# sm-edwards/CrossScale-ECG-A-Modular-HPC-Pipeline-from-Locality-Optimization-to-MPI-GPU-Overlap

Measured on AMD Instinct MI355X. Metric: ECG samples/sec (node) + conv1d speedup vs torch.Conv1d, tiny 1D-CNN at 1/2/4/8 GPU, higher is better.
Workload: dtype bf16; 1 GPU; model=TinyECG (1458 params), global_batch=256, seq_len=500, parallelism=dp1, sync=fedavg every 50 local steps (none all_reduce AVG, overlap=none), per_client_batch=256, max_windows_per_client=20000, backend=fused

## Files before the change

### crossscale-ecg-a-modular-hpc-pipeline-from-locality-optimization-to-mpi-gpu-overlap_amd/ops/_lib.py

```python
from __future__ import annotations

import ctypes as C
import os
import threading
from typing import Optional

import torch

LIB_DIR = os.environ.get("ECG_LIB_DIR") or os.path.join(os.path.dirname(os.path.dirname(os.path.abspath(__file__))), "_lib")

_lock = threading.Lock()
_libs = {}

vp, i32, i64, f32 = C.c_void_p, C.c_int, C.c_long, C.c_float
u64 = C.c_uint64
f64p = C.POINTER(C.c_double)
i32p = C.POINTER(C.c_int)
i64p = C.POINTER(C.c_int64)

STATUS = {0: "ok", 1: "bad argument", 2: "problem too large for the fused kernel", 3: "HIP runtime error",
          4: "I/O error", 5: "timeout", 6: "end of data"}


class NativeError(RuntimeError):
# ... 10 lines not shown
        if name in _libs:
            return _libs[name]
        path = os.path.join(LIB_DIR, name)
        lib = None
        if os.path.exists(path):
            lib = C.CDLL(path, mode=C.RTLD_GLOBAL)
        _libs[name] = lib
        return lib


def _sig(lib, name, argtypes, restype=i32):
    fn = getattr(lib, name)
    fn.argtypes = argtypes
    fn.restype = restype
    return fn


class TinyRound(C.Structure):
    _fields_ = [("X", vp), ("ldx", i64), ("idx", vp), ("Y", vp), ("params", vp), ("mom", vp), ("slab", vp),
                ("loss_acc", vp), ("wprep", vp), ("xg", vp), ("yg", vp),
                ("L", i32), ("nc", i32), ("slab_stride", i32), ("B", i32), ("steps", i32),
                ("lr", f32), ("momentum", f32), ("wd", f32), ("nesterov", i32), ("prec", i32),
                ("dp_clip", f32), ("dp_sigma", f32), ("dp_seed", u64), ("dp_scale", vp), ("dp_step", vp),
                ("xbg", vp)]


class TinyCohortRound(C.Structure):
    _fields_ = [("X", vp), ("ldx", i64), ("idx", vp), ("Y", vp), ("params", vp), ("mom", vp), ("slab", vp),
                ("loss_acc", vp), ("wprep", vp), ("xg", vp), ("yg", vp), ("xbg", vp), ("global_params", vp),
                ("L", i32), ("nc", i32), ("slab_stride", i32), ("B", i32), ("steps", i32), ("M", i32),
                ("fanout", i32), ("lr", f32), ("momentum", f32), ("wd", f32), ("nesterov", i32), ("prec", i32),
                ("cdp_clip", f32), ("cdp_sigma", f32), ("server_lr", f32), ("cdp_seed", u64), ("cdp_scale", vp),
                ("cdp_norm", vp), ("cdp_round", vp), ("server_opt", i32), ("server_beta1", f32), ("server_beta2", f32),
                ("server_tau", f32), ("server_m", vp), ("server_v", vp)]


def _bind_kernels(lib: C.CDLL) -> None:
    _sig(lib, "ecg_tiny_param_count", [i32])
    _sig(lib, "ecg_tiny_smem_bytes", [i32, i32])
    _sig(lib, "ecg_tiny_step_grads", [vp, i32, i64, vp, vp, vp, i32, vp, i32, i32, f32, i32, vp, vp])
    _sig(lib, "ecg_tiny_forward", [vp, i32, i64, vp, vp, i32, vp, i32, i32, vp, vp])
    _sig(lib, "ecg_tiny_wprep_bytes", [])
    _sig(lib, "ecg_tiny_prep", [vp, vp, vp])
    _sig(lib, "ecg_tiny_eval", [vp, i32, i64, vp, vp, i32, vp, i32, vp, vp, vp, vp, vp, i32, vp])
    _sig(lib, "ecg_tiny_eval_scratch_bytes", [i32])
    _sig(lib, "ecg_tiny_eval_out_bytes", [i32])
    _sig(lib, "ecg_slab_reduce_sgd", [vp, i32, i32, i32, vp, vp, vp, vp, f32, f32, f32, i32, i32, vp, vp])
    _sig(lib, "ecg_slab_reduce_dp_sgd", [vp, i32, i32, i32, vp, vp, vp, vp, f32, f32, f32, i32, i32, vp,
                                         f32, f32, u64, vp, vp, vp])
    _sig(lib, "ecg_dp_noise", [vp, i32, u64, u64, vp])
    native = _sig(lib, "ecg_tiny_round_sizeof", [])()
    if native != C.sizeof(TinyRound):
        raise NativeError(f"EcgTinyRound is {native} bytes in libecg_kernels.so but {C.sizeof(TinyRound)} in "
                          "ops/_lib.py: rebuild the library (python csrc/build.py) or update TinyRound")
    _sig(lib, "ecg_tiny_round_enqueue", [C.POINTER(TinyRound), vp])
    _sig(lib, "ecg_tiny_round_capture", [C.POINTER(vp), C.POINTER(TinyRound)])
    native = _sig(lib, "ecg_tiny_cohort_round_sizeof", [])()
    if native != C.sizeof(TinyCohortRound):
        raise NativeError(f"EcgTinyCohortRound is {native} bytes in libecg_kernels.so but {C.sizeof(TinyCohortRound)} "
                          "in ops/_lib.py: rebuild the library (python csrc/build.py) or update TinyCohortRound")
    _sig(lib, "ecg_tiny_cohort_round_enqueue", [C.POINTER(TinyCohortRound), vp])
    _sig(lib, "ecg_tiny_cohort_round_capture", [C.POINTER(vp), C.POINTER(TinyCohortRound)])
    _sig(lib, "ecg_cohort_dp_close", [vp, vp, i32, i32, f32, f32, f32, u64, vp, vp, vp, vp])
    _sig(lib, "ecg_cohort_dp_noise", [vp, i32, u64, u64, vp])
    _sig(lib, "ecg_cohort_server_close", [vp, vp, i32, i32, f32, f32, f32, u64, vp, vp, vp, i32, f32, f32, f32, vp, vp,
                                          vp])
    _sig(lib, "ecg_tiny_cohort_param_stride", [i32])
    _sig(lib, "ecg_tiny_cohort_wprep_stride", [])
    _sig(lib, "ecg_tiny_gather_floats", [i32, i32], i64)
    _sig(lib, "ecg_tiny_gather_halfs", [i32, i32], i64)
    _sig(lib, "ecg_tiny_step_grads_twice", [vp, i32, i64, vp, vp, vp, i32, vp, i32, i32, f32, i32, vp, vp])
    _sig(lib, "ecg_tiny_force_waves", [i32])
    _sig(lib, "ecg_tiny_set_stamps", [vp])
    _sig(lib, "ecg_round_graph_launch", [vp, vp])
    _sig(lib, "ecg_round_graph_destroy", [vp])
    _sig(lib, "ecg_round_graph_upload", [vp, vp])
    _sig(lib, "conv1d_batch_hip", [vp, vp, vp, i32, i32, i32, vp])
    _sig(lib, "conv1d_batch_hip_sync", [vp, vp, vp, i32, i32, i32, vp])
    _sig(lib, "conv1d_batch_hip_spin", [vp, vp, vp, i32, i32, i32, vp])
    _sig(lib, "conv1d_batch_hip_flag", [vp, vp, vp, i32, i32, i32, vp])
    _sig(lib, "conv1d_valid_dgrad_hip", [vp, vp, vp, i32, i32, i32, vp])
    _sig(lib, "conv1d_valid_dgrad_hip_bf16", [vp, vp, vp, i32, i32, i32, vp])
    _sig(lib, "conv1d_valid_wgrad_ws_floats", [i32, i32, i32], i64)
    _sig(lib, "conv1d_valid_wgrad_hip", [vp, vp, vp, vp, i64, i32, i32, i32, vp])
    _sig(lib, "conv1d_valid_wgrad_hip_bf16", [vp, vp, vp, vp, i64, i32, i32, i32, vp])
    _sig(lib, "conv1d_batch_hip_bf16", [vp, vp, vp, i32, i32, i32, vp])
    _sig(lib, "ecg_sgd_flat", [vp, vp, vp, i64, f32, f32, f32, f32, i32, i32, f32, vp, vp])
    _sig(lib, "ecg_gather_rows_f32", [vp, i64, i32, vp, i32, vp, i64, i32, f32, vp])
    _sig(lib, "ecg_gather_rows_bf16", [vp, i64, i32, vp, i32, vp, i64, i32, f32, vp])
    for extra in ("_bind_conv_mc",):
        fn = globals().get(extra)
        if fn:
            fn(lib)
# ... 91 lines not shown
```

### crossscale-ecg-a-modular-hpc-pipeline-from-locality-optimization-to-mpi-gpu-overlap_amd/ops/fused_tiny.py

```python
from __future__ import annotations

import ctypes as C
import os
from typing import Optional

import torch

from . import _lib
from ..models.tiny_ecg import TinyECG, num_params
from ..data.dataset import DeviceIndexSampler
from ..utils.philox import mix64
from .tiny_eval import EvalResult, TinyEvaluator, evaluate_torch, tiny_evaluate


PRECISION = {"bf16": 0, "fp32": 1}


def prec_id(precision: str) -> int:
    if precision not in PRECISION:
        raise ValueError(f"precision must be one of {list(PRECISION)}, got {precision!r}")
    return PRECISION[precision]


def new_wprep(device) -> torch.Tensor:
# ... 49 lines not shown
    _lib.check(st, "ecg_tiny_forward")
    return out


def tiny_step_grads(flat_params: torch.Tensor, x: torch.Tensor, y32: torch.Tensor, idx: Optional[torch.Tensor],
                    batch: int, num_classes: int = 2, slab: Optional[torch.Tensor] = None,
                    precision: str = "bf16", prefrag: bool = True,
                    wprep: Optional[torch.Tensor] = None) -> torch.Tensor:
    _check_dataset(x, y32, num_classes)
    if idx is not None:
        _check_idx(idx, batch, x.shape[0], x.device)
    stride = slab_stride(num_classes)
    if slab is None:
        slab = torch.empty((batch, stride), dtype=torch.float32, device=x.device)
    lib = _lib.kernels()
    wp, _keep = _wprep_ptr(precision, prefrag, x.device, wprep)
    st = lib.ecg_tiny_step_grads(x.data_ptr(), x.shape[1], x.stride(0), _lib.ptr(idx), y32.data_ptr(),
                                 flat_params.data_ptr(), num_classes, slab.data_ptr(), stride, batch,
                                 1.0 / batch, prec_id(precision), wp, _lib.stream_ptr(x.device))
    _lib.check(st, "ecg_tiny_step_grads")
    return slab


def check_dp_args(dp_clip: float, dp_noise: float) -> None:
    if not dp_clip >= 0.0 or not dp_noise >= 0.0:
        raise ValueError(f"dp_clip and dp_noise must be >= 0, got {dp_clip} and {dp_noise}")
    if dp_noise > 0.0 and dp_clip == 0.0:
        raise ValueError("dp_noise > 0 needs a clip norm (dp_clip > 0): the noise is scaled by it")


def dp_reduce_slab(slab: torch.Tensor, dp_clip: float, dp_noise: float, dp_seed: int, dp_step: torch.Tensor,
                   num_classes: int = 2):
    P = num_params(num_classes)
    grad = torch.empty(P, dtype=torch.float32, device=slab.device)
    loss = torch.zeros(1, dtype=torch.float32, device=slab.device)
    scale = torch.empty(slab.shape[0], dtype=torch.float32, device=slab.device)
    st = _lib.kernels().ecg_slab_reduce_dp_sgd(
        slab.data_ptr(), slab.shape[0], slab.stride(0), P, None, None, grad.data_ptr(), loss.data_ptr(), 0.0, 0.0, 0.0,
        0, 0, None, dp_clip, dp_noise, int(dp_seed) & (2 ** 64 - 1), scale.data_ptr(), dp_step.data_ptr(),
        _lib.stream_ptr(slab.device))
    _lib.check(st, "ecg_slab_reduce_dp_sgd")
    return grad, loss, scale


def dp_noise(P: int, seed: int, t: int, device) -> torch.Tensor:
    z = torch.empty(P, dtype=torch.float32, device=device)
    st = _lib.kernels().ecg_dp_noise(z.data_ptr(), P, int(seed) & (2 ** 64 - 1), int(t) & (2 ** 64 - 1),
                                     _lib.stream_ptr(z.device))
    _lib.check(st, "ecg_dp_noise")
    return z


def reduce_slab(slab: torch.Tensor, num_classes: int = 2):
    P = num_params(num_classes)
    grad = torch.empty(P, dtype=torch.float32, device=slab.device)
    loss = torch.zeros(1, dtype=torch.float32, device=slab.device)
    lib = _lib.kernels()
    st = lib.ecg_slab_reduce_sgd(slab.data_ptr(), slab.shape[0], slab.shape[1], P, None, None, grad.data_ptr(),
                                 loss.data_ptr(), 0.0, 0.0, 0.0, 0, 0, None, _lib.stream_ptr(slab.device))
    _lib.check(st, "ecg_slab_reduce_sgd")
    return grad, loss


class FusedTinyTrainer:

    def __init__(self, model: TinyECG, x_gpu: torch.Tensor, y_gpu: torch.Tensor, batch_size: int,
                 steps_per_round: int, lr: float = 1e-2, momentum: float = 0.9, weight_decay: float = 0.0,
                 nesterov: bool = False, seed: Optional[int] = None, use_graph: Optional[bool] = None,
                 precision: str = "bf16", prefrag: bool = True, gather: bool = True, pack: bool = True,
                 dp_clip: float = 0.0, dp_noise: float = 0.0, dp_seed: Optional[int] = None):
        self.device = x_gpu.device
        self.precision = precision
        self.prec = prec_id(precision)
        self.model = model
        self.nc = model.num_classes
        self.params = model.flat if model.flat is not None else model.flatten_parameters()
        if self.params.device != self.device:
            raise ValueError("model and dataset must be on the same device")
        self.P = num_params(self.nc)
        self.x = x_gpu.contiguous()
        self.y32 = labels_int32(y_gpu, self.nc)
        _check_dataset(self.x, self.y32, self.nc)
        self.B = int(batch_size)
        self.S = int(steps_per_round)
        self.lr, self.momentum, self.wd, self.nesterov = float(lr), float(momentum), float(weight_decay), bool(nesterov)
        self.stride = slab_stride(self.nc)
        self.mom = torch.zeros_like(self.params)
        self.slab = torch.empty((self.B, self.stride), dtype=torch.float32, device=self.device)
        self.loss_acc = torch.zeros(1, dtype=torch.float32, device=self.device)
        self.idx_table = torch.zeros((self.S, self.B), dtype=torch.int32, device=self.device)
        self.idx_stage = torch.zeros((self.S, self.B), dtype=torch.int32, device=self.device)
        self._staged: Optional[int] = None
        self._loss_steps = 0
        self.sampler = DeviceIndexSampler(self.x.shape[0], self.B, self.device, seed=seed)
        self.use_graph = (os.environ.get("ECG_TINY_GRAPH", "1") != "0") if use_graph is None else bool(use_graph)
        self._graphs = {}
        self.steps_done = 0
        self._evaluator: Optional[TinyEvaluator] = None
        lib = _lib.kernels()
        L = self.x.shape[1]
        smem = lib.ecg_tiny_smem_bytes(L, self.prec)
        if smem > 160 * 1024:
            raise ValueError(f"window length {L} too long for the fused kernel ({smem} B LDS)")
        self.prefrag = bool(prefrag) and precision == "bf16"
        self.wprep = new_wprep(self.device) if self.prefrag else None
        self.gather = bool(gather) and self.prefrag
        self.xg = self.yg = None
        if self.gather:
            self.xg = torch.zeros(lib.ecg_tiny_gather_floats(L, self.B), dtype=torch.float32, device=self.device)
            self.yg = torch.zeros(2 * self.B, dtype=torch.int32, device=self.device)
        self.pack = bool(pack) and self.gather
        self.xbg = None
        if self.pack:
            self.xbg = torch.zeros(lib.ecg_tiny_gather_halfs(L, self.B), dtype=torch.bfloat16, device=self.device)
        check_dp_args(dp_clip, dp_noise)
        self.dp_clip, self.dp_noise = float(dp_clip), float(dp_noise)
        self.dp = self.dp_clip > 0.0
        self.dp_seed = (mix64(0 if seed is None else seed) if dp_seed is None else int(dp_seed)) & (2 ** 64 - 1)
        self.dp_steps = 0
        self.dp_scale = self.dp_step = None
        if self.dp:
            self.dp_scale = torch.zeros(self.B, dtype=torch.float32, device=self.device)
            self.dp_step = torch.zeros(1, dtype=torch.int64, device=self.device)
        self._round = _lib.TinyRound(
            X=self.x.data_ptr(), ldx=self.x.stride(0), Y=self.y32.data_ptr(), params=self.params.data_ptr(),
            mom=self.mom.data_ptr(), slab=self.slab.data_ptr(), loss_acc=self.loss_acc.data_ptr(),
            wprep=_lib.ptr(self.wprep), xg=_lib.ptr(self.xg), yg=_lib.ptr(self.yg), L=L, nc=self.nc,
            slab_stride=self.stride, B=self.B, lr=self.lr, momentum=self.momentum, wd=self.wd,
            nesterov=int(self.nesterov), prec=self.prec, dp_clip=self.dp_clip, dp_sigma=self.dp_noise,
            dp_seed=self.dp_seed, dp_scale=_lib.ptr(self.dp_scale), dp_step=_lib.ptr(self.dp_step),
            xbg=_lib.ptr(self.xbg))

    def _round_of(self, n: int, table: torch.Tensor):
        r = self._round
        r.idx, r.steps = table.data_ptr(), n
        return C.byref(r)

    def _graph_for(self, n: int, table: torch.Tensor) -> C.c_void_p:
        key = (n, table.data_ptr())
        g = self._graphs.get(key)
        if g is None:
            g = C.c_void_p()
            torch.cuda.synchronize(self.device)
            _lib.check(_lib.kernels().ecg_tiny_round_capture(C.byref(g), self._round_of(n, table)),
                       "ecg_tiny_round_capture")
            self._graphs[key] = g
        return g

    def close(self):
        graphs, self._graphs = getattr(self, "_graphs", {}), {}
        for g in graphs.values():
            if g.value:
                _lib.kernels().ecg_round_graph_destroy(g)

# ... 100 lines not shown
```

### csrc/kernels/tiny_ecg_step.hip

```cpp
#include "../include/ecg_common.h"
#include "../include/tiny_ecg.h"

#include <cfloat>
#include <climits>
#include <cstdint>
#include <cstdlib>
#include <cstring>
#include <type_traits>

namespace {

using namespace ecg::tiny;

constexpr int MAX_PAIRS_PER_WAVE = 4;

struct Smem {
  int Lp;
  int xs_off, xcol_off, h1_off, dh2_off, ps_off, frag_off, red_off, bytes;
};

constexpr int RED_G = 0;
constexpr int RED_POOLED = 16;
constexpr int RED_POOL = 48;

struct FusedOpt {
  int slab_wt;
};
__host__ __device__ constexpr int msplit(int waves) { return (waves - 1) / 5 < 1 ? 1 : (waves - 1) / 5; }
__host__ __device__ constexpr int red_cnt(int waves) { return RED_POOL + waves * 16; }
__host__ __device__ constexpr int red_m(int waves) { return red_cnt(waves) + waves * 16; }
__host__ __device__ constexpr int red_dw1(int waves) { return red_m(waves) + msplit(waves) * 1280; }
__host__ __device__ constexpr int red_head(int waves) { return red_dw1(waves) + waves * 128; }
__host__ __device__ constexpr int red_floats(int waves) { return red_head(waves) + 288; }

typedef unsigned u32x4 __attribute__((ext_vector_type(4)));
typedef unsigned u32x2 __attribute__((ext_vector_type(2)));

__device__ __forceinline__ void st_wt(__amdgpu_buffer_rsrc_t r, int idx, float v) {
  __builtin_amdgcn_raw_buffer_store_b32(__builtin_bit_cast(unsigned, v), r, idx * 4, 0, 16);
}
__device__ __forceinline__ void st_wt4(__amdgpu_buffer_rsrc_t r, int idx, f32x4 v) {
  typedef int i32x4 __attribute__((ext_vector_type(4)));
  __builtin_amdgcn_raw_buffer_store_b128(__builtin_bit_cast(i32x4, v), r, idx * 4, 0, 16);
}
__device__ __forceinline__ void st_wt_b64(__amdgpu_buffer_rsrc_t r, int byte_off, u32x2 v) {
  __builtin_amdgcn_raw_buffer_store_b64(v, r, byte_off, 0, 16);
}
__device__ __forceinline__ void st_wt_b16(__amdgpu_buffer_rsrc_t r, int byte_off, unsigned short v) {
  __builtin_amdgcn_raw_buffer_store_b16(v, r, byte_off, 0, 16);
}
__device__ __forceinline__ float ld_wt(__amdgpu_buffer_rsrc_t r, int idx) {
  return __builtin_bit_cast(float, __builtin_amdgcn_raw_buffer_load_b32(r, idx * 4, 0, 16));
}
constexpr int kOobByte = 0x40000000;

constexpr int kPackLead = 4;
__host__ __device__ constexpr int pack_ldb(int L) { return (L + 31) / 32 * 32 + 8; }

constexpr int F32_KSTEPS = C * K2 / 4;

__host__ __device__ constexpr bool frag_pad_is_bias(int which, int l, int j) { return which == 0 && j == 0 && l < 48; }

__device__ __forceinline__ void wprep_put(unsigned char* wp, int i, float v) {
  __bf16* wb = reinterpret_cast<__bf16*>(wp);
  if (i < C * K1) {
    wb[WP_AW1 + (i / K1) * 8 + i % K1] = ecg::to_bf16(v);
// ... 714 lines not shown
    }
  }
};

__host__ __device__ constexpr int cohort_pstride(int P) { return (P + 63) / 64 * 64; }
constexpr int kCohortWprepStride = (WP_BYTES + 127) / 128 * 128;

template <int WAVES, int MODE, bool F32, bool PF, bool PK = false>
__global__ __launch_bounds__(WAVES * 64) void tiny_ecg_step_kernel(
    const float* __restrict__ X, long ldx,
    const unsigned char* __restrict__ wprep,
    const int* __restrict__ Y,
    unsigned long long* __restrict__ stamps,
    int L, int nc,
    const float* __restrict__ params,
    float* __restrict__ out, int out_stride,
    float inv_B,
    const int* __restrict__ idx,
    int slab_wt) {
  extern __shared__ __attribute__((aligned(16))) unsigned char smem[];
  TinySample<WAVES, F32, PF, PK> S(smem, L, nc);
  constexpr bool TRAIN = MODE != 1;
  constexpr bool COHORT = MODE == 3;
  const int tid = threadIdx.x;
  const int b = COHORT ? blockIdx.y * gridDim.x + blockIdx.x : blockIdx.x;
  const long rows = COHORT ? (long)gridDim.x * gridDim.y : (long)gridDim.x;
  if constexpr (COHORT) {
    params += (long)blockIdx.y * cohort_pstride(S.lay.P);
    if constexpr (PF) wprep += (long)blockIdx.y * kCohortWprepStride;
  }
  const __amdgpu_buffer_rsrc_t slab_r = make_rsrc(out, rows * out_stride * 4);
  const int rowbase = b * out_stride;
  if (stamps && tid == 0) stamps[(long)b * 16 + 15] = __builtin_amdgcn_s_memrealtime();
#pragma unroll 1
  for (int rep = 0; rep < (MODE == 2 ? 2 : 1); ++rep) {
#define ECG_STAMP(k) \
  if (stamps && tid == 0) stamps[(long)b * 16 + 7 * rep + (k)] = __builtin_amdgcn_s_memtime();
    ECG_STAMP(0)
    int ylab = 0;
    long row = b;
    if constexpr (!PK) row = idx ? (long)idx[b] : (long)b;
    const float* xrow = X + row * ldx;
    [[maybe_unused]] const __amdgpu_buffer_rsrc_t xr = make_rsrc(xrow, PK ? ldx * 4 : (long)L * 4);
    [[maybe_unused]] typename TinySample<WAVES, F32, PF, PK>::X1 x0;
    [[maybe_unused]] float hv_pk = 0.f;
    if constexpr (PK) {
      S.conv1_load(xr, 0, x0);
      ylab = Y[row];
      S.pf_load_fwd(wprep);
      const int i = S.lay.wh + tid;
      hv_pk = i < S.lay.P ? params[i] : 0.f;
    } else if constexpr (PF) {
      S.pf_load_fwd(wprep);
      const int i = S.lay.wh + tid;
      const float hv = i < S.lay.P ? params[i] : 0.f;
      if (TRAIN) ylab = Y[row];
      S.conv1_load(xr, 0, x0);
      if (i < S.lay.P) S.ps[i] = hv;
      static_assert(MAX_CLASSES * C + MAX_CLASSES <= 8 * 64, "head parameters: one per thread");
    } else {
      constexpr int PR = 4;
      float pv[PR];
#pragma unroll
      for (int j = 0; j < PR; ++j) {
        const int i = tid + j * S.NT;
        pv[j] = i < S.lay.P ? params[i] : 0.f;
// ... 13 lines not shown
      for (int i = tid + PR * S.NT; i < S.lay.P; i += S.NT) S.put_param(i, params[i]);
    }
    S.zero_pads();
    if constexpr (F32) {
      __syncthreads();
      ECG_STAMP(1)
      S.conv1();
    } else {
      ECG_STAMP(1)
      S.conv1_mfma(xr, x0);
      if constexpr (PK) {
        const int i = S.lay.wh + tid;
        if (i < S.lay.P) S.ps[i] = hv_pk;
      }
    }
    __syncthreads();
    ECG_STAMP(2)
    S.conv2();
    if constexpr (PF && TRAIN) S.pf_load_dgrad(wprep);
    __syncthreads();
    ECG_STAMP(3)
    S.template head_and_M<TRAIN>(ylab, inv_B, out, out_stride, b);
    if (!TRAIN) return;
    if (MODE == 0 && stamps && (tid & 63) == 0 && (S.w <= 1 || S.w == WAVES - 1))
      stamps[(long)b * 16 + 8 + (S.w == 0 ? 0 : S.w == 1 ? 1 : 2)] = __builtin_amdgcn_s_memtime();
    __syncthreads();
    ECG_STAMP(4)
    S.dgrad();
    __syncthreads();
    ECG_STAMP(5)
    if (WAVES == 16 && slab_wt && S.lay.P - S.lay.b2 + 1 <= S.NT - 448) {
      S.row_store(slab_r, rowbase);
    } else if (slab_wt) {
      for (int i = tid; i <= S.lay.P; i += S.NT) st_wt(slab_r, rowbase + i, S.row_value(i));
    } else {
      for (int i = tid; i <= S.lay.P; i += S.NT) out[rowbase + i] = S.row_value(i);
    }
    ECG_STAMP(6)
#undef ECG_STAMP
    if (MODE == 2) __syncthreads();
  }
  if (stamps && tid == 0) stamps[(long)b * 16 + 14] = __builtin_amdgcn_s_memrealtime();
}

constexpr int kRedColsDefault = 32;
constexpr int kRedApply = 1, kRedNesterov = 2;
inline int red_flags(int apply, int nesterov) { return (apply ? kRedApply : 0) | (nesterov ? kRedNesterov : 0); }
constexpr int RED_ROWG = 16;

struct GatherArgs {
  const float* X;
  long ldx;
  const int* idx;
  const int* Y;
  float* xg;
  int* yg;
  int L, ldg, B, vec;
  __bf16* xbg;
  int ldb;
};
__host__ __device__ inline int gather_rows_per_block(int L, int vec, int nt) {
  const int per_row = vec ? L / 4 : L;
  return per_row >= nt ? 1 : nt / per_row;
}

template <int NT>
__device__ __forceinline__ void gather_block(const GatherArgs& ga, int nred) {
  const int per_row = ga.vec ? ga.L / 4 : ga.L;
  const int rpb = gather_rows_per_block(ga.L, ga.vec, NT);
  const int r0 = ((int)blockIdx.x - nred) * rpb;
  const __amdgpu_buffer_rsrc_t xr = make_rsrc(ga.xg, (long)ga.B * ga.ldg * 4);
  const __amdgpu_buffer_rsrc_t br = make_rsrc(ga.xbg, ga.xbg ? (long)ga.B * ga.ldb * 2 : 0);
  const int npad = ga.ldb - ga.L;
  for (int e = threadIdx.x; e < rpb * per_row; e += NT) {
    const int lr_ = e / per_row, j = e - lr_ * per_row, b = r0 + lr_;
    if (b >= ga.B) break;
    const long row = ga.idx[b];
    if (ga.vec) {
      const f32x4 v = *reinterpret_cast<const f32x4*>(ga.X + row * ga.ldx + 4 * j);
      st_wt4(xr, b * ga.ldg + 4 * j, v);
      if (ga.xbg) {
        bf16x4 p;
#pragma unroll
        for (int q = 0; q < 4; ++q) p[q] = ecg::to_bf16(v[q]);
        st_wt_b64(br, (b * ga.ldb + kPackLead + 4 * j) * 2, __builtin_bit_cast(u32x2, p));
        for (int u = j; u < npad / 4; u += per_row)
          st_wt_b64(br, (b * ga.ldb + (u == 0 ? 0 : ga.L + 4 * u)) * 2, u32x2{0u, 0u});
      }
    } else {
      const float v = ga.X[row * ga.ldx + j];
      st_wt(xr, b * ga.ldg + j, v);
      if (ga.xbg) {
        st_wt_b16(br, (b * ga.ldb + kPackLead + j) * 2, __builtin_bit_cast(unsigned short, ecg::to_bf16(v)));
        for (int u = j; u < npad; u += per_row)
          st_wt_b16(br, (b * ga.ldb + (u < kPackLead ? u : ga.L + u)) * 2, (unsigned short)0);
// ... 231 lines not shown
  if (lane == 0) {
    const float n = sqrtf(ss);
    norm[c] = n;
    scale[c] = n > 0.f ? fminf(1.f, clip / n) : 1.f;
  }
}

template <int NT>
__global__ __launch_bounds__(NT) void cohort_dp_mean_kernel(
    const float* __restrict__ params, float* __restrict__ global_params, int P, int M, float inv_M,
    const float* __restrict__ scale, float server_lr, float noise_scale, unsigned long long seed,
    const unsigned long long* __restrict__ round_word) {
  const int i = blockIdx.x * NT + threadIdx.x;
  if (i >= P) return;
  const int pstride = cohort_pstride(P);
  float noise = 0.f;
  if (noise_scale != 0.f) noise = noise_scale * cohort_dp_normal(i, seed, round_word[0] - 1ull);
  const float g = global_params[i];
  float s = scale[0] * (params[i] - g);
  for (int c = 1; c < M; ++c) s += scale[c] * (params[(long)c * pstride + i] - g);
  global_params[i] = g + server_lr * (s * inv_M + noise);
}

unsigned long long* g_stamps = nullptr;

FusedOpt no_fuse() {
  FusedOpt o{};
  o.slab_wt = 1;
  return o;
}

struct StepArgs {
  const float* X;
  int L;
  long ldx;
  const int* idx;
  const int* Y;
  const float* params;
  int nc;
  float* out;
  int out_stride, B;
  float inv_B;
  const unsigned char* wprep;
  bool packed = false;
};

template <int WAVES, int MODE, bool F32, bool PF, bool PK = false>
int launch_step(const StepArgs& a, hipStream_t stream, int M = 1) {
  const Smem sm = make_smem(a.L, WAVES, a.nc, F32);
  auto kern = tiny_ecg_step_kernel<WAVES, MODE, F32, PF, PK>;
  if (sm.bytes > 64 * 1024)
    ECG_HIP_CHECK(hipFuncSetAttribute((const void*)kern, hipFuncAttributeMaxDynamicSharedMemorySize, sm.bytes));
  if (PK && a.idx) return ecg::kBadArg;
  hipLaunchKernelGGL(kern, dim3(a.B, M), dim3(WAVES * 64), sm.bytes, stream, a.X, a.ldx, PF ? a.wprep : nullptr, a.Y,
                     g_stamps, a.L, a.nc, a.params, a.out, a.out_stride, a.inv_B, a.idx, no_fuse().slab_wt);
  ECG_HIP_CHECK(hipGetLastError());
  return ecg::kOk;
}

int launch_prep(const float* params, unsigned char* wprep, hipStream_t stream) {
  if (!params || !wprep) return ecg::kBadArg;
  hipLaunchKernelGGL(tiny_prep_kernel, dim3(1), dim3(256), 0, stream, params, wprep);
  ECG_HIP_CHECK(hipGetLastError());
  return ecg::kOk;
}

constexpr int kMaxLds = 160 * 1024;

int g_forced_waves = 0;
int pick_waves(int L, bool f32) {
  const int Lp = (L + 31) / 32 * 32;
  const int forced = g_forced_waves;
  const bool fit16 = Lp <= 32 * 4 * 16 && make_smem(L, 16, MAX_CLASSES, f32).bytes <= kMaxLds;
  if (forced == 16 && fit16) return 16;
  if (forced == 8) return 8;
  return (fit16 && Lp / 32 >= 16) ? 16 : 8;
}
// ... 3 lines not shown
  const int Lp = (L + 31) / 32 * 32;
  if (Lp > 32 * 4 * 8 || make_smem(L, 8, MAX_CLASSES, f32).bytes > kMaxLds) return ecg::kTooLarge;
  const Layout lay = make_layout(nc);
  if (mode != 1 && out_stride < lay.P + 1) return ecg::kBadArg;
  if (mode == 1 && out_stride < nc) return ecg::kBadArg;
  return ecg::kOk;
}

template <bool F32, bool PF>
int dispatch_cfg(int mode, int waves, const StepArgs& a, hipStream_t stream) {
  if (mode == 2)
    return launch_step<8, 2, F32, PF>(a, stream);
  if (mode == 0) return waves == 8 ? launch_step<8, 0, F32, PF>(a, stream) : launch_step<16, 0, F32, PF>(a, stream);
  return waves == 8 ? launch_step<8, 1, F32, PF>(a, stream) : launch_step<16, 1, F32, PF>(a, stream);
}

int step_dispatch(int mode, int prec, const StepArgs& a, hipStream_t stream) {
  if (prec != 0 && prec != 1) return ecg::kBadArg;
  int st = check_step_args(a.L, a.nc, a.B, a.out_stride, mode, prec == 1);
  if (st) return st;
  if (a.wprep && prec == 1) return ecg::kBadArg;
  const int waves = pick_waves(a.L, prec == 1);
  if (a.packed) {
    if (mode != 0 || prec != 0 || !a.wprep || a.idx) return ecg::kBadArg;
    return waves == 8 ? launch_step<8, 0, false, true, true>(a, stream)
                      : launch_step<16, 0, false, true, true>(a, stream);
  }
  if (prec == 1) return dispatch_cfg<true, false>(mode, waves, a, stream);
  if (a.wprep) return dispatch_cfg<false, true>(mode, waves, a, stream);
  return dispatch_cfg<false, false>(mode, waves, a, stream);
}

int check_reduce(int G, int stride, int P, int apply, const float* params, float momentum, const float* mom) {
  if (G <= 0 || P <= 0 || stride < P + 1) return ecg::kBadArg;
  if (apply && (!params || (momentum != 0.f && !mom))) return ecg::kBadArg;
  return ecg::kOk;
}

constexpr int kRedThreads = kRedColsDefault * RED_ROWG;
struct RedGeom {
  int blocks, nred, grid;
  GatherArgs ga;
};
RedGeom red_geom(int P, int M, const GatherArgs* gather, bool cohort = false) {
  RedGeom g{(P + kRedColsDefault) / kRedColsDefault, 0, 0, {}};
  g.grid = M * g.blocks;
  g.nred = (gather || cohort) ? g.grid : INT_MAX;
  if (gather) {
    g.ga = *gather;
    const int rpb = gather_rows_per_block(g.ga.L, g.ga.vec, kRedThreads);
    g.grid += (g.ga.B + rpb - 1) / rpb;
  }
  return g;
}

int reduce_dispatch(const float* slab, int G, int stride, int P, float* params, float* mom, float* grad_out,
                    float* loss_acc, float lr, float momentum, float wd, int nesterov, int apply,
                    unsigned char* wprep, hipStream_t stream, const GatherArgs* gather = nullptr) {
  const int st = check_reduce(G, stride, P, apply, params, momentum, mom);
  if (st) return st;
  const RedGeom g = red_geom(P, 1, gather);
  hipLaunchKernelGGL(slab_reduce_sgd_kernel<kRedColsDefault>, dim3(g.grid), dim3(kRedThreads), 0, stream, slab, params,
                     mom, g.nred, G, stride, P, red_flags(apply, nesterov), momentum, lr, wd, wprep, loss_acc, grad_out,
                     g.ga);
  ECG_HIP_CHECK(hipGetLastError());
  return ecg::kOk;
}

struct DpArgs {
  float clip, sigma;
  unsigned long long seed;
  float* scale;
  unsigned long long* step;
// ... 106 lines not shown
  return ecg::kOk;
}

struct EcgTinyRound {
  const float* X;
  long ldx;
  const int* idx;
  const int* Y;
  float* params;
  float* mom;
  float* slab;
  float* loss_acc;
  void* wprep;
  float* xg;
  int* yg;
  int L, nc, slab_stride, B, steps;
  float lr, momentum, wd;
  int nesterov, prec;
  float dp_clip, dp_sigma;
  unsigned long long dp_seed;
  float* dp_scale;
  unsigned long long* dp_step;
  void* xbg;
};

ECG_API int ecg_tiny_round_sizeof(void) { return (int)sizeof(EcgTinyRound); }

static int check_round(const EcgTinyRound* r) {
  if (!r || r->steps < 1 || !r->X || !r->Y || !r->params || !r->slab) return ecg::kBadArg;
  if (r->prec != 0 && r->prec != 1) return ecg::kBadArg;
  if (r->wprep && r->prec != 0) return ecg::kBadArg;
  if ((!r->xg) != (!r->yg) || (r->xg && (!r->wprep || !r->idx))) return ecg::kBadArg;
  if (r->xbg && !r->xg) return ecg::kBadArg;
  if (r->dp_clip < 0.f || r->dp_sigma < 0.f || (r->dp_sigma > 0.f && r->dp_clip == 0.f)) return ecg::kBadArg;
  if (r->dp_clip > 0.f && (!r->dp_scale || !r->dp_step)) return ecg::kBadArg;
  return check_step_args(r->L, r->nc, r->B, r->slab_stride, 0, r->prec == 1);
}

struct GatherBufs {
  float* xg;
  int* yg;
  __bf16* xbg;
};
static GatherArgs gather_args(const float* X, long ldx, const int* Y, int L, int rows) {
  const int vec = (L % 4 == 0 && ldx % 4 == 0 && reinterpret_cast<uintptr_t>(X) % 16 == 0) ? 1 : 0;
  return {X, ldx, nullptr, Y, nullptr, nullptr, L, (L + 3) / 4 * 4, rows, vec, nullptr, pack_ldb(L)};
}
static void gather_fill(GatherArgs& ga, const GatherBufs& g, int s, const int* idx_next) {
  const long buf = (long)((s + 1) & 1) * ga.B;
  ga.idx = idx_next;
  ga.xg = g.xg + buf * ga.ldg;
  ga.yg = g.yg + buf;
  ga.xbg = g.xbg ? g.xbg + buf * ga.ldb : nullptr;
}
static void gather_read(StepArgs& a, const GatherArgs& ga, const GatherBufs& g, int s) {
  const long buf = (long)(s & 1) * ga.B;
  a.X = g.xg + buf * ga.ldg;
  a.ldx = ga.ldg;
  a.idx = nullptr;
  a.Y = g.yg + buf;
  if (g.xbg) {
    a.X = reinterpret_cast<const float*>(g.xbg + buf * ga.ldb);
    a.ldx = ga.ldb / 2;
    a.packed = true;
  }
}

static int enqueue_round(const EcgTinyRound& r, hipStream_t stream) {
  const int P = make_layout(r.nc).P;
  unsigned char* wprep = static_cast<unsigned char*>(r.wprep);
  const GatherBufs bufs{r.xg, r.yg, static_cast<__bf16*>(r.xbg)};
  GatherArgs ga = gather_args(r.X, r.ldx, r.Y, r.L, r.B);
  for (int s = 0; s < r.steps; ++s) {
    const int* idx = r.idx ? r.idx + (long)s * r.B : nullptr;
    const bool gather_next = r.xg && s + 1 < r.steps;
    if (gather_next) gather_fill(ga, bufs, s, idx + r.B);
    StepArgs a{r.X, r.L, r.ldx, idx, r.Y, r.params, r.nc, r.slab, r.slab_stride, r.B, 1.0f / (float)r.B,
               s == 0 ? nullptr : wprep};
    if (r.xg && s > 0) gather_read(a, ga, bufs, s);
    int st = step_dispatch(0, r.prec, a, stream);
    if (st) return st;
    if (r.dp_clip > 0.f)
      st = dp_reduce_dispatch(r.slab, r.B, r.slab_stride, P, r.params, r.mom, nullptr, r.loss_acc, r.lr, r.momentum,
                              r.wd, r.nesterov, 1, wprep, {r.dp_clip, r.dp_sigma, r.dp_seed, r.dp_scale, r.dp_step},
                              stream, gather_next ? &ga : nullptr);
    else
      st = reduce_dispatch(r.slab, r.B, r.slab_stride, P, r.params, r.mom, nullptr, r.loss_acc, r.lr, r.momentum, r.wd,
                           r.nesterov, 1, wprep, stream, gather_next ? &ga : nullptr);
    if (st) return st;
  }
  return ecg::kOk;
}

template <class Enqueue>
static int capture_round(void** handle, int steps, Enqueue enqueue) {
  hipStream_t cap;
  ECG_HIP_CHECK(hipStreamCreateWithFlags(&cap, hipStreamNonBlocking));
  RoundGraph* rg = new RoundGraph();
  rg->steps = steps;
  hipError_t e = hipStreamBeginCapture(cap, hipStreamCaptureModeThreadLocal);
  if (e != hipSuccess) {
    delete rg;
// ... 13 lines not shown
    (void)hipGraphDestroy(rg->graph);
    delete rg;
    return ecg::kHipError;
  }
  *handle = rg;
  return ecg::kOk;
}

ECG_API int ecg_tiny_round_enqueue(const EcgTinyRound* round, hipStream_t stream) {
  const int st = check_round(round);
  return st ? st : enqueue_round(*round, stream);
}

ECG_API int ecg_tiny_round_capture(void** handle, const EcgTinyRound* round) {
  if (!handle) return ecg::kBadArg;
  const int st = check_round(round);
  if (st) return st;
  return capture_round(handle, round->steps, [&](hipStream_t cap) { return enqueue_round(*round, cap); });
}

ECG_API long ecg_tiny_gather_floats(int L, int B) { return 2L * B * ((L + 3) / 4 * 4); }

ECG_API long ecg_tiny_gather_halfs(int L, int B) { return 2L * B * pack_ldb(L); }

ECG_API int ecg_round_graph_launch(void* handle, hipStream_t stream) {
  if (!handle) return ecg::kBadArg;
  RoundGraph* rg = static_cast<RoundGraph*>(handle);
  ECG_HIP_CHECK(hipGraphLaunch(rg->exec, stream));
  return ecg::kOk;
}

ECG_API int ecg_round_graph_upload(void* handle, hipStream_t stream) {
  if (!handle) return ecg::kBadArg;
  RoundGraph* rg = static_cast<RoundGraph*>(handle);
  ECG_HIP_CHECK(hipGraphUpload(rg->exec, stream));
  return ecg::kOk;
}

ECG_API int ecg_round_graph_destroy(void* handle) {
  if (!handle) return ecg::kOk;
  RoundGraph* rg = static_cast<RoundGraph*>(handle);
  if (rg->exec) (void)hipGraphExecDestroy(rg->exec);
  if (rg->graph) (void)hipGraphDestroy(rg->graph);
  delete rg;
  return ecg::kOk;
}
// ... 269 lines not shown
```

Baseline: 26.92 million samples/s.

## Prepack dataset to padded bf16 once and read packed rows directly in step kernel

Adds a one-time kernel that converts the whole fp32 training shard into padded bf16 rows, plus a new step-kernel mode that indexes those packed rows through the sample indices. The default 'direct' mode drops the per-step gather/convert pass and its double-buffered staging. The gather blocks are no longer added to the reduce kernel, and no fp32 staging buffer is needed. The cost is extra device memory for the packed copy, limited to a share of free memory with a fallback to the old path. The packed copy must also be refreshed if the dataset changes.

```diff
diff --git a/crossscale-ecg-a-modular-hpc-pipeline-from-locality-optimization-to-mpi-gpu-overlap_amd/ops/_lib.py b/crossscale-ecg-a-modular-hpc-pipeline-from-locality-optimization-to-mpi-gpu-overlap_amd/ops/_lib.py
--- a/crossscale-ecg-a-modular-hpc-pipeline-from-locality-optimization-to-mpi-gpu-overlap_amd/ops/_lib.py
+++ b/crossscale-ecg-a-modular-hpc-pipeline-from-locality-optimization-to-mpi-gpu-overlap_amd/ops/_lib.py
@@ -56,7 +56,10 @@
                 ("L", i32), ("nc", i32), ("slab_stride", i32), ("B", i32), ("steps", i32),
                 ("lr", f32), ("momentum", f32), ("wd", f32), ("nesterov", i32), ("prec", i32),
                 ("dp_clip", f32), ("dp_sigma", f32), ("dp_seed", u64), ("dp_scale", vp), ("dp_step", vp),
-                ("xbg", vp)]
+                ("xbg", vp), ("xpk", vp), ("prepack", i32)]
+
+
+PREPACK = {"none": 0, "gather": 1, "direct": 2}
 
 
 class TinyCohortRound(C.Structure):
@@ -103,6 +106,8 @@
     _sig(lib, "ecg_tiny_cohort_wprep_stride", [])
     _sig(lib, "ecg_tiny_gather_floats", [i32, i32], i64)
     _sig(lib, "ecg_tiny_gather_halfs", [i32, i32], i64)
+    _sig(lib, "ecg_tiny_pack_halfs", [i32, i64], i64)
+    _sig(lib, "ecg_tiny_pack_dataset", [vp, i64, i64, i32, vp, vp])
     _sig(lib, "ecg_tiny_step_grads_twice", [vp, i32, i64, vp, vp, vp, i32, vp, i32, i32, f32, i32, vp, vp])
     _sig(lib, "ecg_tiny_force_waves", [i32])
     _sig(lib, "ecg_tiny_set_stamps", [vp])
diff --git a/crossscale-ecg-a-modular-hpc-pipeline-from-locality-optimization-to-mpi-gpu-overlap_amd/ops/fused_tiny.py b/crossscale-ecg-a-modular-hpc-pipeline-from-locality-optimization-to-mpi-gpu-overlap_amd/ops/fused_tiny.py
--- a/crossscale-ecg-a-modular-hpc-pipeline-from-locality-optimization-to-mpi-gpu-overlap_amd/ops/fused_tiny.py
+++ b/crossscale-ecg-a-modular-hpc-pipeline-from-locality-optimization-to-mpi-gpu-overlap_amd/ops/fused_tiny.py
@@ -95,6 +95,36 @@
     return slab
 
 
+PREPACK_DEFAULT = "direct"
+PREPACK_SHARE = 0.25
+
+
+def _prepack_variant(prepack, explicit_gather: bool = False) -> str:
+    if prepack is None:
+        prepack = "none" if explicit_gather else os.environ.get("ECG_TINY_PREPACK") or PREPACK_DEFAULT
+    if prepack is True:
+        prepack = "gather" if PREPACK_DEFAULT == "none" else PREPACK_DEFAULT
+    if prepack is False:
+        prepack = "none"
+    if prepack not in _lib.PREPACK:
+        raise ValueError(f"prepack must be a bool or one of {list(_lib.PREPACK)}, got {prepack!r}")
+    return prepack
+
+
+def pack_dataset(x: torch.Tensor, out: Optional[torch.Tensor] = None) -> torch.Tensor:
+    _check_dataset(x, None, 0)
+    lib = _lib.kernels()
+    N, L = x.shape
+    ldb = lib.ecg_tiny_pack_halfs(L, 1)
+    if out is None:
+        out = torch.empty((N, ldb), dtype=torch.bfloat16, device=x.device)
+    if out.shape != (N, ldb) or out.dtype != torch.bfloat16 or not out.is_contiguous() or out.device != x.device:
+        raise ValueError(f"packed rows must be a contiguous bfloat16 [{N}, {ldb}] tensor on the dataset's device")
+    _lib.check(lib.ecg_tiny_pack_dataset(x.data_ptr(), x.stride(0), N, L, out.data_ptr(), _lib.stream_ptr(x.device)),
+               "ecg_tiny_pack_dataset")
+    return out
+
+
 def check_dp_args(dp_clip: float, dp_noise: float) -> None:
     if not dp_clip >= 0.0 or not dp_noise >= 0.0:
         raise ValueError(f"dp_clip and dp_noise must be >= 0, got {dp_clip} and {dp_noise}")
@@ -140,7 +170,9 @@
     def __init__(self, model: TinyECG, x_gpu: torch.Tensor, y_gpu: torch.Tensor, batch_size: int,
                  steps_per_round: int, lr: float = 1e-2, momentum: float = 0.9, weight_decay: float = 0.0,
                  nesterov: bool = False, seed: Optional[int] = None, use_graph: Optional[bool] = None,
-                 precision: str = "bf16", prefrag: bool = True, gather: bool = True, pack: bool = True,
+                 precision: str = "bf16", prefrag: bool = True, gather: Optional[bool] = None,
+                 pack: Optional[bool] = None,
+                 prepack=None, prepack_share: float = PREPACK_SHARE,
                  dp_clip: float = 0.0, dp_noise: float = 0.0, dp_seed: Optional[int] = None):
         self.device = x_gpu.device
         self.precision = precision
@@ -177,15 +209,22 @@
             raise ValueError(f"window length {L} too long for the fused kernel ({smem} B LDS)")
         self.prefrag = bool(prefrag) and precision == "bf16"
         self.wprep = new_wprep(self.device) if self.prefrag else None
-        self.gather = bool(gather) and self.prefrag
-        self.xg = self.yg = None
-        if self.gather:
-            self.xg = torch.zeros(lib.ecg_tiny_gather_floats(L, self.B), dtype=torch.float32, device=self.device)
+        explicit_gather = gather is not None or pack is not None
+        self.gather = (True if gather is None else bool(gather)) and self.prefrag
+        self.pack = (True if pack is None else bool(pack)) and self.gather
+        self.prepack_share = float(prepack_share)
+        self.prepack, self.prepack_fallback = _prepack_variant(prepack, explicit_gather) if self.pack else "none", None
+        self.xpk = None
+        if self.prepack != "none":
+            self._alloc_prepacked()
+        self.xg = self.yg = self.xbg = None
+        if self.gather and self.prepack != "direct":
             self.yg = torch.zeros(2 * self.B, dtype=torch.int32, device=self.device)
-        self.pack = bool(pack) and self.gather
-        self.xbg = None
-        if self.pack:
-            self.xbg = torch.zeros(lib.ecg_tiny_gather_halfs(L, self.B), dtype=torch.bfloat16, device=self.device)
+            if self.prepack == "none":
+                self.xg = torch.zeros(lib.ecg_tiny_gather_floats(L, self.B), dtype=torch.float32, device=self.device)
+            if self.pack:
+                self.xbg = torch.zeros(lib.ecg_tiny_gather_halfs(L, self.B), dtype=torch.bfloat16,
+                                       device=self.device)
         check_dp_args(dp_clip, dp_noise)
         self.dp_clip, self.dp_noise = float(dp_clip), float(dp_noise)
         self.dp = self.dp_clip > 0.0
@@ -202,7 +241,27 @@
             slab_stride=self.stride, B=self.B, lr=self.lr, momentum=self.momentum, wd=self.wd,
             nesterov=int(self.nesterov), prec=self.prec, dp_clip=self.dp_clip, dp_sigma=self.dp_noise,
             dp_seed=self.dp_seed, dp_scale=_lib.ptr(self.dp_scale), dp_step=_lib.ptr(self.dp_step),
-            xbg=_lib.ptr(self.xbg))
+            xbg=_lib.ptr(self.xbg), xpk=_lib.ptr(self.xpk), prepack=_lib.PREPACK[self.prepack])
+
+    def _alloc_prepacked(self) -> None:
+        N, L = self.x.shape
+        need = 2 * _lib.kernels().ecg_tiny_pack_halfs(L, N)
+        free, _total = torch.cuda.mem_get_info(self.device)
+        if need > self.prepack_share * free:
+            self.prepack_fallback = (f"packed shard of {need} B exceeds {self.prepack_share:g} of the {free} B free")
+        else:
+            try:
+                self.xpk = torch.empty((N, need // (2 * N)), dtype=torch.bfloat16, device=self.device)
+            except torch.cuda.OutOfMemoryError as e:
+                self.prepack_fallback = f"allocation of {need} B failed: {e}"
+        if self.xpk is None:
+            self.prepack = "none"
+        else:
+            self.repack()
+
+    def repack(self) -> None:
+        if self.xpk is not None:
+            pack_dataset(self.x, self.xpk)
 
     def _round_of(self, n: int, table: torch.Tensor):
         r = self._round
diff --git a/csrc/kernels/tiny_ecg_step.hip b/csrc/kernels/tiny_ecg_step.hip
--- a/csrc/kernels/tiny_ecg_step.hip
+++ b/csrc/kernels/tiny_ecg_step.hip
@@ -42,6 +42,10 @@
 __device__ __forceinline__ void st_wt4(__amdgpu_buffer_rsrc_t r, int idx, f32x4 v) {
   typedef int i32x4 __attribute__((ext_vector_type(4)));
   __builtin_amdgcn_raw_buffer_store_b128(__builtin_bit_cast(i32x4, v), r, idx * 4, 0, 16);
+}
+__device__ __forceinline__ void st_wt_b128(__amdgpu_buffer_rsrc_t r, int byte_off, u32x4 v) {
+  typedef int i32x4 __attribute__((ext_vector_type(4)));
+  __builtin_amdgcn_raw_buffer_store_b128(__builtin_bit_cast(i32x4, v), r, byte_off, 0, 16);
 }
 __device__ __forceinline__ void st_wt_b64(__amdgpu_buffer_rsrc_t r, int byte_off, u32x2 v) {
   __builtin_amdgcn_raw_buffer_store_b64(v, r, byte_off, 0, 16);
@@ -802,6 +806,8 @@
   TinySample<WAVES, F32, PF, PK> S(smem, L, nc);
   constexpr bool TRAIN = MODE != 1;
   constexpr bool COHORT = MODE == 3;
+  constexpr bool PKI = MODE == 4;
+  static_assert(!PKI || PK, "MODE 4 reads packed rows");
   const int tid = threadIdx.x;
   const int b = COHORT ? blockIdx.y * gridDim.x + blockIdx.x : blockIdx.x;
   const long rows = COHORT ? (long)gridDim.x * gridDim.y : (long)gridDim.x;
@@ -819,9 +825,16 @@
     ECG_STAMP(0)
     int ylab = 0;
     long row = b;
-    if constexpr (!PK) row = idx ? (long)idx[b] : (long)b;
-    const float* xrow = X + row * ldx;
-    [[maybe_unused]] const __amdgpu_buffer_rsrc_t xr = make_rsrc(xrow, PK ? ldx * 4 : (long)L * 4);
+    long pitch = ldx;
+    if constexpr (PKI) {
+      typedef const __attribute__((address_space(4))) int* IdxPtr;
+      row = ((IdxPtr)ldx)[b];
+      pitch = pack_ldb(L) / 2;
+    } else if constexpr (!PK) {
+      row = idx ? (long)idx[b] : (long)b;
+    }
+    const float* xrow = X + row * pitch;
+    [[maybe_unused]] const __amdgpu_buffer_rsrc_t xr = make_rsrc(xrow, PK ? pitch * 4 : (long)L * 4);
     [[maybe_unused]] typename TinySample<WAVES, F32, PF, PK>::X1 x0;
     [[maybe_unused]] float hv_pk = 0.f;
     if constexpr (PK) {
@@ -881,7 +894,7 @@
     ECG_STAMP(3)
     S.template head_and_M<TRAIN>(ylab, inv_B, out, out_stride, b);
     if (!TRAIN) return;
-    if (MODE == 0 && stamps && (tid & 63) == 0 && (S.w <= 1 || S.w == WAVES - 1))
+    if ((MODE == 0 || PKI) && stamps && (tid & 63) == 0 && (S.w <= 1 || S.w == WAVES - 1))
       stamps[(long)b * 16 + 8 + (S.w == 0 ? 0 : S.w == 1 ? 1 : 2)] = __builtin_amdgcn_s_memtime();
     __syncthreads();
     ECG_STAMP(4)
@@ -917,19 +930,33 @@
   int L, ldg, B, vec;
   __bf16* xbg;
   int ldb;
+  const __bf16* xpk;
 };
-__host__ __device__ inline int gather_rows_per_block(int L, int vec, int nt) {
-  const int per_row = vec ? L / 4 : L;
+__host__ __device__ inline int gather_per_row(const GatherArgs& ga) {
+  return ga.xpk ? ga.ldb / 8 : ga.vec ? ga.L / 4 : ga.L;
+}
+__host__ __device__ inline int gather_rows_per_block(int per_row, int nt) {
   return per_row >= nt ? 1 : nt / per_row;
 }
 
 template <int NT>
 __device__ __forceinline__ void gather_block(const GatherArgs& ga, int nred) {
-  const int per_row = ga.vec ? ga.L / 4 : ga.L;
-  const int rpb = gather_rows_per_block(ga.L, ga.vec, NT);
+  const int per_row = gather_per_row(ga);
+  const int rpb = gather_rows_per_block(per_row, NT);
   const int r0 = ((int)blockIdx.x - nred) * rpb;
+  const __amdgpu_buffer_rsrc_t br = make_rsrc(ga.xbg, ga.xbg ? (long)ga.B * ga.ldb * 2 : 0);
+  if (ga.xpk) {
+    for (int e = threadIdx.x; e < rpb * per_row; e += NT) {
+      const int lr_ = e / per_row, j = e - lr_ * per_row, b = r0 + lr_;
+      if (b >= ga.B) break;
+      const long row = ga.idx[b];
+      const u32x4 v = *reinterpret_cast<const u32x4*>(ga.xpk + row * ga.ldb + 8 * j);
+      st_wt_b128(br, (b * ga.ldb + 8 * j) * 2, v);
+      if (j == 0) ga.yg[b] = ga.Y[row];
+    }
+    return;
+  }
   const __amdgpu_buffer_rsrc_t xr = make_rsrc(ga.xg, (long)ga.B * ga.ldg * 4);
-  const __amdgpu_buffer_rsrc_t br = make_rsrc(ga.xbg, ga.xbg ? (long)ga.B * ga.ldb * 2 : 0);
   const int npad = ga.ldb - ga.L;
   for (int e = threadIdx.x; e < rpb * per_row; e += NT) {
     const int lr_ = e / per_row, j = e - lr_ * per_row, b = r0 + lr_;
@@ -1207,6 +1234,38 @@
   global_params[i] = g + server_lr * (s * inv_M + noise);
 }
 
+template <bool VEC>
+__global__ __launch_bounds__(128) void tiny_pack_rows_kernel(const float* __restrict__ X, long ldx, long N, int L,
+                                                             __bf16* __restrict__ out) {
+  const int ldb = pack_ldb(L);
+  for (long n = blockIdx.x; n < N; n += gridDim.x) {
+    const float* x = X + n * ldx;
+    __bf16* o = out + n * ldb;
+    if constexpr (VEC) {
+      for (int u = threadIdx.x; u < ldb / 4; u += blockDim.x) {
+        const int j = 4 * u - kPackLead;
+        bf16x4 p;
+        if (j >= 0 && j < L) {
+          const f32x4 v = *reinterpret_cast<const f32x4*>(x + j);
+#pragma unroll
+          for (int q = 0; q < 4; ++q) p[q] = ecg::to_bf16(v[q]);
+        } else {
+#pragma unroll
+          for (int q = 0; q < 4; ++q) p[q] = ecg::to_bf16(0.f);
+        }
+        *reinterpret_cast<bf16x4*>(o + 4 * u) = p;
+      }
+    } else {
+      for (int e = threadIdx.x; e < ldb; e += blockDim.x) {
+        const int j = e - kPackLead;
+        const bool in = j >= 0 && j < L;
+        const unsigned short v = __builtin_bit_cast(unsigned short, ecg::to_bf16(x[in ? j : 0]));
+        reinterpret_cast<unsigned short*>(o)[e] = in ? v : (unsigned short)0;
+      }
+    }
+  }
+}
+
 unsigned long long* g_stamps = nullptr;
 
 FusedOpt no_fuse() {
@@ -1236,8 +1295,9 @@
   auto kern = tiny_ecg_step_kernel<WAVES, MODE, F32, PF, PK>;
   if (sm.bytes > 64 * 1024)
     ECG_HIP_CHECK(hipFuncSetAttribute((const void*)kern, hipFuncAttributeMaxDynamicSharedMemorySize, sm.bytes));
-  if (PK && a.idx) return ecg::kBadArg;
-  hipLaunchKernelGGL(kern, dim3(a.B, M), dim3(WAVES * 64), sm.bytes, stream, a.X, a.ldx, PF ? a.wprep : nullptr, a.Y,
+  if (PK && (MODE == 4) != (a.idx != nullptr)) return ecg::kBadArg;
+  const long ldx = MODE == 4 ? (long)reinterpret_cast<uintptr_t>(a.idx) : a.ldx;
+  hipLaunchKernelGGL(kern, dim3(a.B, M), dim3(WAVES * 64), sm.bytes, stream, a.X, ldx, PF ? a.wprep : nullptr, a.Y,
                      g_stamps, a.L, a.nc, a.params, a.out, a.out_stride, a.inv_B, a.idx, no_fuse().slab_wt);
   ECG_HIP_CHECK(hipGetLastError());
   return ecg::kOk;
@@ -1287,9 +1347,12 @@
   if (a.wprep && prec == 1) return ecg::kBadArg;
   const int waves = pick_waves(a.L, prec == 1);
   if (a.packed) {
-    if (mode != 0 || prec != 0 || !a.wprep || a.idx) return ecg::kBadArg;
-    return waves == 8 ? launch_step<8, 0, false, true, true>(a, stream)
-                      : launch_step<16, 0, false, true, true>(a, stream);
+    if (mode != 0 || prec != 0 || !a.wprep) return ecg::kBadArg;
+    if (!a.idx)
+      return waves == 8 ? launch_step<8, 0, false, true, true>(a, stream)
+                        : launch_step<16, 0, false, true, true>(a, stream);
+    return waves == 8 ? launch_step<8, 4, false, true, true>(a, stream)
+                      : launch_step<16, 4, false, true, true>(a, stream);
   }
   if (prec == 1) return dispatch_cfg<true, false>(mode, waves, a, stream);
   if (a.wprep) return dispatch_cfg<false, true>(mode, waves, a, stream);
@@ -1313,7 +1376,7 @@
   g.nred = (gather || cohort) ? g.grid : INT_MAX;
   if (gather) {
     g.ga = *gather;
-    const int rpb = gather_rows_per_block(g.ga.L, g.ga.vec, kRedThreads);
+    const int rpb = gather_rows_per_block(gather_per_row(g.ga), kRedThreads);
     g.grid += (g.ga.B + rpb - 1) / rpb;
   }
   return g;
@@ -1466,7 +1529,10 @@
   float* dp_scale;
   unsigned long long* dp_step;
   void* xbg;
+  const void* xpk;
+  int prepack;
 };
+enum { kPrepackNone = 0, kPrepackGather = 1, kPrepackDirect = 2 };
 
 ECG_API int ecg_tiny_round_sizeof(void) { return (int)sizeof(EcgTinyRound); }
 
@@ -1474,8 +1540,17 @@
   if (!r || r->steps < 1 || !r->X || !r->Y || !r->params || !r->slab) return ecg::kBadArg;
   if (r->prec != 0 && r->prec != 1) return ecg::kBadArg;
   if (r->wprep && r->prec != 0) return ecg::kBadArg;
-  if ((!r->xg) != (!r->yg) || (r->xg && (!r->wprep || !r->idx))) return ecg::kBadArg;
-  if (r->xbg && !r->xg) return ecg::kBadArg;
+  if (r->prepack == kPrepackNone) {
+    if (r->xpk) return ecg::kBadArg;
+    if ((!r->xg) != (!r->yg) || (r->xg && (!r->wprep || !r->idx))) return ecg::kBadArg;
+    if (r->xbg && !r->xg) return ecg::kBadArg;
+  } else {
+    if (r->prepack != kPrepackGather && r->prepack != kPrepackDirect) return ecg::kBadArg;
+    if (!r->xpk || !r->wprep || !r->idx || r->xg) return ecg::kBadArg;
+    const bool bufs = r->prepack == kPrepackGather;
+    if ((r->yg != nullptr) != bufs || (r->xbg != nullptr) != bufs) return ecg::kBadArg;
+    if (reinterpret_cast<uintptr_t>(r->xpk) % 16 != 0) return ecg::kBadArg;
+  }
   if (r->dp_clip < 0.f || r->dp_sigma < 0.f || (r->dp_sigma > 0.f && r->dp_clip == 0.f)) return ecg::kBadArg;
   if (r->dp_clip > 0.f && (!r->dp_scale || !r->dp_step)) return ecg::kBadArg;
   return check_step_args(r->L, r->nc, r->B, r->slab_stride, 0, r->prec == 1);
@@ -1485,21 +1560,23 @@
   float* xg;
   int* yg;
   __bf16* xbg;
+  const __bf16* xpk = nullptr;
 };
 static GatherArgs gather_args(const float* X, long ldx, const int* Y, int L, int rows) {
   const int vec = (L % 4 == 0 && ldx % 4 == 0 && reinterpret_cast<uintptr_t>(X) % 16 == 0) ? 1 : 0;
-  return {X, ldx, nullptr, Y, nullptr, nullptr, L, (L + 3) / 4 * 4, rows, vec, nullptr, pack_ldb(L)};
+  return {X, ldx, nullptr, Y, nullptr, nullptr, L, (L + 3) / 4 * 4, rows, vec, nullptr, pack_ldb(L), nullptr};
 }
 static void gather_fill(GatherArgs& ga, const GatherBufs& g, int s, const int* idx_next) {
   const long buf = (long)((s + 1) & 1) * ga.B;
   ga.idx = idx_next;
-  ga.xg = g.xg + buf * ga.ldg;
+  ga.xg = g.xg ? g.xg + buf * ga.ldg : nullptr;
   ga.yg = g.yg + buf;
   ga.xbg = g.xbg ? g.xbg + buf * ga.ldb : nullptr;
+  ga.xpk = g.xpk;
 }
 static void gather_read(StepArgs& a, const GatherArgs& ga, const GatherBufs& g, int s) {
   const long buf = (long)(s & 1) * ga.B;
-  a.X = g.xg + buf * ga.ldg;
+  a.X = g.xg ? g.xg + buf * ga.ldg : nullptr;
   a.ldx = ga.ldg;
   a.idx = nullptr;
   a.Y = g.yg + buf;
@@ -1513,15 +1590,21 @@
 static int enqueue_round(const EcgTinyRound& r, hipStream_t stream) {
   const int P = make_layout(r.nc).P;
   unsigned char* wprep = static_cast<unsigned char*>(r.wprep);
-  const GatherBufs bufs{r.xg, r.yg, static_cast<__bf16*>(r.xbg)};
+  const __bf16* xpk = static_cast<const __bf16*>(r.xpk);
+  const bool gathers = r.xg || r.prepack == kPrepackGather;
+  const GatherBufs bufs{r.xg, r.yg, static_cast<__bf16*>(r.xbg), r.prepack == kPrepackGather ? xpk : nullptr};
   GatherArgs ga = gather_args(r.X, r.ldx, r.Y, r.L, r.B);
   for (int s = 0; s < r.steps; ++s) {
     const int* idx = r.idx ? r.idx + (long)s * r.B : nullptr;
-    const bool gather_next = r.xg && s + 1 < r.steps;
+    const bool gather_next = gathers && s + 1 < r.steps;
     if (gather_next) gather_fill(ga, bufs, s, idx + r.B);
     StepArgs a{r.X, r.L, r.ldx, idx, r.Y, r.params, r.nc, r.slab, r.slab_stride, r.B, 1.0f / (float)r.B,
                s == 0 ? nullptr : wprep};
-    if (r.xg && s > 0) gather_read(a, ga, bufs, s);
+    if (gathers && s > 0) gather_read(a, ga, bufs, s);
+    if (r.prepack == kPrepackDirect && s > 0) {
+      a.X = reinterpret_cast<const float*>(xpk);
+      a.packed = true;
+    }
     int st = step_dispatch(0, r.prec, a, stream);
     if (st) return st;
     if (r.dp_clip > 0.f)
@@ -1581,6 +1664,21 @@
 ECG_API long ecg_tiny_gather_floats(int L, int B) { return 2L * B * ((L + 3) / 4 * 4); }
 
 ECG_API long ecg_tiny_gather_halfs(int L, int B) { return 2L * B * pack_ldb(L); }
+
+ECG_API long ecg_tiny_pack_halfs(int L, long N) { return N * pack_ldb(L); }
+
+ECG_API int ecg_tiny_pack_dataset(const float* X, long ldx, long N, int L, void* out, hipStream_t stream) {
+  if (!X || !out || N <= 0 || L < 1 || ldx < L || reinterpret_cast<uintptr_t>(out) % 16 != 0) return ecg::kBadArg;
+  const bool vec = L % 4 == 0 && ldx % 4 == 0 && reinterpret_cast<uintptr_t>(X) % 16 == 0;
+  const unsigned grid = (unsigned)(N < (1L << 20) ? N : (1L << 20));
+  __bf16* o = static_cast<__bf16*>(out);
+  if (vec)
+    hipLaunchKernelGGL(tiny_pack_rows_kernel<true>, dim3(grid), dim3(128), 0, stream, X, ldx, N, L, o);
+  else
+    hipLaunchKernelGGL(tiny_pack_rows_kernel<false>, dim3(grid), dim3(128), 0, stream, X, ldx, N, L, o);
+  ECG_HIP_CHECK(hipGetLastError());
+  return ecg::kOk;
+}
 
 ECG_API int ecg_round_graph_launch(void* handle, hipStream_t stream) {
   if (!handle) return ecg::kBadArg;
```

New measurement: 27.78 million samples/s, median of 6. 3.2% higher.
